# zkMIPS/zkm

Hardware: AMD Instinct MI355X
Metric: segment_proofs_per_sec (higher is better)
Workload: dtype u64 (Goldilocks p = 2^64 - 2^32 + 1, integer modular)

## Files before the change

### zkm_amd/csrc/gl_dev.h

```cpp
#pragma once
#include <stdint.h>

#if defined(__HIPCC__)
#include <hip/hip_runtime.h>
#define GL_HD __host__ __device__ __forceinline__
#else
#define GL_HD inline
#endif

typedef uint64_t gl_t;

static constexpr uint64_t GL_P = 0xFFFFFFFF00000001ULL;
static constexpr uint64_t GL_EPS = 0xFFFFFFFFULL;
static constexpr uint64_t GL_GENERATOR = 14293326489335486720ULL;
static constexpr uint64_t GL_POW2_GENERATOR = 7277203076849721926ULL;

GL_HD gl_t gl_canon(uint64_t x) { return x >= GL_P ? x - GL_P : x; }

GL_HD gl_t gl_add(gl_t a, gl_t b) {
    uint64_t s = a + b;
    return (s < a || s >= GL_P) ? s - GL_P : s;
}
GL_HD gl_t gl_sub(gl_t a, gl_t b) { return a >= b ? a - b : a - b + GL_P; }
GL_HD gl_t gl_neg(gl_t a) { return a ? GL_P - a : 0; }
// ... 71 lines not shown
    return d;
}
#endif

template <uint32_t IMM>
GL_HD uint64_t gl_mad_imm(uint32_t x, uint64_t c) {
    static_assert(IMM <= 64, "gl_mad_imm: the multiplier must be an inline constant");
#if defined(__HIP_DEVICE_COMPILE__)
    uint64_t r, carry;
    asm("v_mad_u64_u32 %0, %1, %2, %3, %4" : "=v"(r), "=s"(carry) : "v"(x), "n"(IMM), "v"(c));
    return r;
#else
    return (uint64_t)x * IMM + c;
#endif
}
template <uint32_t IMM>
GL_HD uint64_t gl_mad_imm_sc(uint32_t x, uint64_t c) {
    static_assert(IMM <= 64, "gl_mad_imm_sc: the multiplier must be an inline constant");
#if defined(__HIP_DEVICE_COMPILE__)
    uint64_t r, carry;
    asm("v_mad_u64_u32 %0, %1, %2, %3, %4" : "=v"(r), "=s"(carry) : "v"(x), "n"(IMM), "s"(c));
    return r;
#else
    return (uint64_t)x * IMM + c;
#endif
}
GL_HD uint64_t gl_mad_s(uint32_t x, uint32_t m, uint64_t c) {
#if defined(__HIP_DEVICE_COMPILE__)
    uint64_t r, carry;
    asm("v_mad_u64_u32 %0, %1, %2, %3, %4" : "=v"(r), "=s"(carry) : "v"(x), "s"(m), "v"(c));
    return r;
#else
    return (uint64_t)x * m + c;
#endif
}

GL_HD uint64_t gl_reduce128(uint64_t lo, uint64_t hi) {
    uint32_t h1 = (uint32_t)(hi >> 32), h0 = (uint32_t)hi;
#if defined(__HIP_DEVICE_COMPILE__) && !defined(GL_REDUCE_BRANCHFREE)
    uint32_t tl, th;
    uint64_t bm;
    asm("v_sub_co_u32 %0, vcc, %3, %5\n\tv_subbrev_co_u32 %1, vcc, 0, %4, vcc\n\ts_mov_b64 %2, vcc"
        : "=&v"(tl), "=&v"(th), "=s"(bm)
        : "v"((uint32_t)lo), "v"((uint32_t)(lo >> 32)), "v"(h1)
        : "vcc");
    uint64_t t0 = ((uint64_t)th << 32) | tl;
    if (__builtin_expect(bm != 0, 0)) {
        asm volatile("; ZKM_COLD");
        if ((bm >> (__lane_id() & 63)) & 1) t0 -= GL_EPS;
    }
#else
    uint64_t t0 = lo - h1;
    uint32_t m = (uint32_t)((int32_t)((uint32_t)(t0 >> 32) & ~(uint32_t)(lo >> 32)) >> 31);
    t0 -= m;
#endif
#if defined(__HIP_DEVICE_COMPILE__)
    uint64_t r, carry;
    uint32_t wrap;
    asm("v_mad_u64_u32 %0, %1, %3, -1, %4\n\ts_nop 1\n\tv_cndmask_b32 %2, 0, -1, %1" : "=&v"(r), "=&s"(carry), "=v"(wrap) : "v"(h0), "v"(t0));
    return r + wrap;
#else
    uint64_t r = (uint64_t)h0 * 0xFFFFFFFFu + t0;
    r += (r < t0) ? GL_EPS : 0;
    return r;
#endif
}
// ... 176 lines not shown
```

### zkm_amd/csrc/hash.hip

```cpp
#include <atomic>
#include "poseidon_dev.h"
#include "poseidon_lat_dev.h"
#include "poseidon_mfma_dev.h"
#include "hash_constants_dev.h"
#include "zkm_internal.h"

#ifndef ZKM_LEAF_MFMA_WAVES
#define ZKM_LEAF_MFMA_WAVES (ZKM_MFMA_PARK ? 5 : 4)
#endif

#ifndef ZKM_LATENCY_PRIO
#define ZKM_LATENCY_PRIO 3
#endif
#define ZKM_RAISE_PRIO()                                              \
    do {                                                              \
        if (ZKM_LATENCY_PRIO) __builtin_amdgcn_s_setprio(ZKM_LATENCY_PRIO); \
    } while (0)

__global__ __launch_bounds__(256) void k_poseidon_permute(gl_t* states, size_t k) {
    size_t i = (size_t)blockIdx.x * blockDim.x + threadIdx.x;
    if (i >= k) return;
    uint64_t s[12];
#pragma unroll
    for (int j = 0; j < 12; j++) s[j] = states[i * 12 + j];
    poseidon_permute(s);
#pragma unroll
    for (int j = 0; j < 12; j++) states[i * 12 + j] = s[j];
}

void zkm_launch_poseidon_permute(zkm_ctx* c, gl_t* states, size_t k) {
    if (!k) return;
    zkm_prof_scope ps(c, "poseidon_permute");
    hipLaunchKernelGGL(k_poseidon_permute, dim3((k + 255) / 256), dim3(256), 0, c->stream, states, k);
    ZKM_HIP_CHECK(hipGetLastError());
}

struct leaf_cols {
    static constexpr bool WHOLE = false;
    const gl_t* lde;
    size_t ncols, col_stride, seg;
    __device__ __forceinline__ void seek(size_t k) { lde += (size_t)blockIdx.z * seg; lde += k; }
    __device__ __forceinline__ size_t words() const { return ncols; }
    __device__ __forceinline__ uint64_t word(size_t m) const { return lde[m * col_stride]; }
};
struct leaf_f2 {
    static constexpr bool WHOLE = true;
    const gl_t* c0;
    const gl_t* c1;
    unsigned arity;
    size_t seg;
    __device__ __forceinline__ void seek(size_t k) {
        c0 += (size_t)blockIdx.z * seg; c1 += (size_t)blockIdx.z * seg;
        c0 += k * arity; c1 += k * arity;
    }
    __device__ __forceinline__ unsigned words() const { return 2 * arity; }
    __device__ __forceinline__ uint64_t word(unsigned m) const {
        const gl_t *a = c0, *b = c1;
        return ((m & 1) ? b : a)[m >> 1];
    }
};


template <class MDS>
struct sponge_lane {
    static constexpr unsigned LANES = 1;
    static constexpr bool MFMA = std::is_same<MDS, poseidon_mds_mfma>::value;
    typedef uint64_t state_t[12];
    MDS mds;
    size_t item;
    bool live;
    __device__ __forceinline__ sponge_lane() {
        if constexpr (MFMA) {
            mds.A = poseidon_mfma_operand();
#if ZKM_MFMA_PARK
            __shared__ uint32_t park[24 * ZKM_MFMA_PARK_STRIDE];
            mds.park = park + threadIdx.x;
#endif
        }
    }
    __device__ __forceinline__ bool take(size_t n) {
        item = (size_t)blockIdx.x * blockDim.x + threadIdx.x;
        live = item < n;
        if (!MFMA && !live) return false;
        if (!live) item = n - 1;
        return true;
    }
    __device__ __forceinline__ void clear(state_t& s) const {
#pragma unroll
        for (int i = 0; i < 12; i++) s[i] = 0;
    }
    template <bool RAGGED, class Src, class I>
    __device__ __forceinline__ void load(state_t& s, const Src& src, I c, I n) const {
        if (!RAGGED) {
            uint64_t v[8];
#pragma unroll
            for (int i = 0; i < 8; i++) v[i] = src.word(c + i);
#pragma unroll
            for (int i = 0; i < 8; i++) s[i] = v[i];
        } else {
#pragma unroll
            for (int i = 0; i < 8; i++)
                if ((I)i < n - c) s[i] = src.word(c + i);
        }
    }
    __device__ __forceinline__ void permute(state_t& s, int out) const { poseidon_permute_out_t(s, out, mds); }
    template <class Src>
    __device__ __forceinline__ void copy(state_t& s, const Src& src) const {
        for (size_t c = 0; c < src.words(); c++) s[c] = src.word(c);
    }
    template <class K>
    __device__ __forceinline__ void store_digest(const state_t& s, uint64_t* digests, K k, bool on) const {
        if (!on) return;
        uint64_t* d = digests + 4 * k;
        *reinterpret_cast<ulonglong2*>(d) = make_ulonglong2(s[0], s[1]);
        *reinterpret_cast<ulonglong2*>(d + 2) = make_ulonglong2(s[2], s[3]);
    }
    __device__ __forceinline__ void load_state(state_t& s, const gl_t* __restrict__ state, size_t n) const {
#pragma unroll
        for (int i = 0; i < 12; i++) s[i] = state[(size_t)i * n + item];
    }
    __device__ __forceinline__ void store_state(const state_t& s, gl_t* __restrict__ state, size_t n) const {
        if (!live) return;
#pragma unroll
        for (int i = 0; i < 12; i++) state[(size_t)i * n + item] = s[i];
    }
};

using sponge_lane_valu = sponge_lane<poseidon_mds_valu>;
using sponge_lane_mfma = sponge_lane<poseidon_mds_mfma>;

struct sponge_quad {
    static constexpr unsigned LANES = 4;
    typedef uint64_t state_t[3];
    const poseidon_quad Q;
    const unsigned q;
    size_t item;
    bool live;
    __device__ __forceinline__ sponge_quad() : Q(threadIdx.x, table()), q(threadIdx.x & 3) {}
// ... 26 lines not shown
        if (on) digests[4 * k + q] = s[0];
    }
};

struct sponge_wide {
    static constexpr unsigned LANES = 16;
    typedef uint64_t state_t[1];
    const unsigned lane, idx;
    size_t item;
    bool live;
    __device__ __forceinline__ sponge_wide() : lane(threadIdx.x & 63), idx(lane & 15) {}
    __device__ __forceinline__ bool take(size_t n) {
        item = ((size_t)blockIdx.x * blockDim.x + threadIdx.x) >> 4;
        live = item < n;
        return true;
    }
    __device__ __forceinline__ void clear(state_t& s) const { s[0] = 0; }
    template <bool RAGGED, class Src, class I>
    __device__ __forceinline__ void load(state_t& s, const Src& src, I c, I n) const {
        if (live && idx < 8 && (!RAGGED || c + idx < n)) s[0] = src.word(c + idx);
    }
    __device__ __forceinline__ void permute(state_t& s, int) const { s[0] = poseidon_permute_wide(s[0], lane); }
    template <class K>
    __device__ __forceinline__ void compress(state_t& s, const uint64_t* nodes, K k, bool on) const {
        s[0] = (on && idx < 8) ? nodes[8 * k + idx] : 0;
        permute(s, POSEIDON_OUT_DIGEST);
    }
    template <class K>
    __device__ __forceinline__ void store_digest(const state_t& s, uint64_t* digests, K k, bool on) const {
        if (on && idx < 4) digests[4 * k + idx] = s[0];
    }
};

template <class Form, class Src, bool CHUNK = false>
__device__ __forceinline__ void merkle_leaves_body(Src src, size_t n, gl_t* __restrict__ digests, size_t dig_seg, gl_t* __restrict__ state = nullptr,
                                                   int first = 1, int last = 1) {
    Form f;
    if (!f.take(n)) return;
    src.seek(f.item);
    digests += (size_t)blockIdx.z * dig_seg;
    typename Form::state_t s;
    if constexpr (CHUNK) {
        if (first) f.clear(s);
        else f.load_state(s, state, n);
    } else {
        f.clear(s);
    }
    const auto nw = src.words();
    constexpr bool NOOP = Form::LANES == 1 && !CHUNK && !Src::WHOLE;
    if (NOOP && nw <= 4) {
        if constexpr (NOOP) f.copy(s, src);
    } else {
        decltype(src.words()) c = 0;
        for (; CHUNK ? c + 8 <= nw : c < nw; c += 8) {
            if (Src::WHOLE || CHUNK || (Form::LANES == 1 && nw - c >= 8)) f.template load<false>(s, src, c, nw);
            else f.template load<true>(s, src, c, nw);
            f.permute(s, c + 16 <= nw ? POSEIDON_OUT_CAPACITY : ((Src::WHOLE || c + 8 >= nw) && !CHUNK ? POSEIDON_OUT_DIGEST : POSEIDON_OUT_ALL));
        }
        if constexpr (CHUNK) {
            if (c < nw) {
                f.template load<true>(s, src, c, nw);
                sponge_lane_valu().permute(s, POSEIDON_OUT_ALL);
            }
        }
    }
    if constexpr (CHUNK) {
        if (!last) {
            f.store_state(s, state, n);
            return;
        }
    }
    f.store_digest(s, digests, f.item, f.live);
}

#define ZKM_LEAF_MFMA_ATTR __attribute__((amdgpu_waves_per_eu(ZKM_LEAF_MFMA_WAVES, ZKM_LEAF_MFMA_WAVES)))
#define ZKM_LANE_WAVES_ATTR(n) __attribute__((amdgpu_waves_per_eu(n, n)))

__global__ __launch_bounds__(256) ZKM_LANE_WAVES_ATTR(5) void k_merkle_leaves(const gl_t* __restrict__ lde, size_t nrows, size_t ncols, size_t col_stride,
                                                       gl_t* __restrict__ digests, size_t lde_seg, size_t dig_seg) {
    merkle_leaves_body<sponge_lane_valu>(leaf_cols{lde, ncols, col_stride, lde_seg}, nrows, digests, dig_seg);
}
__global__ __launch_bounds__(256) ZKM_LEAF_MFMA_ATTR void k_merkle_leaves_mfma(const gl_t* __restrict__ lde, size_t nrows, size_t ncols, size_t col_stride,
                                                                              gl_t* __restrict__ digests, size_t lde_seg, size_t dig_seg) {
    merkle_leaves_body<sponge_lane_mfma>(leaf_cols{lde, ncols, col_stride, lde_seg}, nrows, digests, dig_seg);
}
__global__ __launch_bounds__(256) void k_merkle_leaves_quad(const gl_t* __restrict__ lde, size_t nrows, size_t ncols, size_t col_stride,
                                                            gl_t* __restrict__ digests, size_t lde_seg, size_t dig_seg) {
    ZKM_RAISE_PRIO();
    merkle_leaves_body<sponge_quad>(leaf_cols{lde, ncols, col_stride, lde_seg}, nrows, digests, dig_seg);
}
__global__ __launch_bounds__(256) void k_merkle_leaves_wide(const gl_t* __restrict__ lde, size_t nrows, size_t ncols, size_t col_stride,
                                                            gl_t* __restrict__ digests, size_t lde_seg, size_t dig_seg) {
    ZKM_RAISE_PRIO();
    merkle_leaves_body<sponge_wide>(leaf_cols{lde, ncols, col_stride, lde_seg}, nrows, digests, dig_seg);
}

__global__ __launch_bounds__(256) void k_merkle_leaves_chunk(const gl_t* __restrict__ lde, size_t nrows, size_t nc, size_t col_stride,
                                                             gl_t* __restrict__ state, int first, int last, gl_t* __restrict__ digests) {
    merkle_leaves_body<sponge_lane_valu, leaf_cols, true>(leaf_cols{lde, nc, col_stride, 0}, nrows, digests, 0, state, first, last);
}
__global__ __launch_bounds__(256) ZKM_LEAF_MFMA_ATTR void k_merkle_leaves_chunk_mfma(const gl_t* __restrict__ lde, size_t nrows, size_t nc, size_t col_stride,
                                                                                    gl_t* __restrict__ state, int first, int last, gl_t* __restrict__ digests) {
    merkle_leaves_body<sponge_lane_mfma, leaf_cols, true>(leaf_cols{lde, nc, col_stride, 0}, nrows, digests, 0, state, first, last);
}

__global__ __launch_bounds__(256) ZKM_LANE_WAVES_ATTR(5) void k_merkle_leaves_ext(const gl_t* __restrict__ c0, const gl_t* __restrict__ c1,
                                                           size_t nleaves, unsigned arity, gl_t* __restrict__ digests, size_t val_seg, size_t dig_seg) {
    merkle_leaves_body<sponge_lane_valu>(leaf_f2{c0, c1, arity, val_seg}, nleaves, digests, dig_seg);
}
__global__ __launch_bounds__(256) ZKM_LEAF_MFMA_ATTR void k_merkle_leaves_ext_mfma(const gl_t* __restrict__ c0, const gl_t* __restrict__ c1, size_t nleaves,
                                                                                  unsigned arity, gl_t* __restrict__ digests, size_t val_seg, size_t dig_seg) {
    merkle_leaves_body<sponge_lane_mfma>(leaf_f2{c0, c1, arity, val_seg}, nleaves, digests, dig_seg);
}
__global__ __launch_bounds__(256) void k_merkle_leaves_ext_quad(const gl_t* __restrict__ c0, const gl_t* __restrict__ c1, size_t nleaves,
                                                                unsigned arity, gl_t* __restrict__ digests, size_t val_seg, size_t dig_seg) {
    ZKM_RAISE_PRIO();
    merkle_leaves_body<sponge_quad>(leaf_f2{c0, c1, arity, val_seg}, nleaves, digests, dig_seg);
}
__global__ __launch_bounds__(256) void k_merkle_leaves_ext_wide(const gl_t* __restrict__ c0, const gl_t* __restrict__ c1, size_t nleaves,
                                                                unsigned arity, gl_t* __restrict__ digests, size_t val_seg, size_t dig_seg) {
    ZKM_RAISE_PRIO();
    merkle_leaves_body<sponge_wide>(leaf_f2{c0, c1, arity, val_seg}, nleaves, digests, dig_seg);
}

enum merkle_form { MERKLE_LANE, MERKLE_LANE_MFMA, MERKLE_QUAD, MERKLE_WIDE };
static merkle_form merkle_pick_form(const zkm_ctx* c, size_t hashes, bool mfma_ok) {
    if (hashes <= c->wide_max_hashes) return MERKLE_WIDE;
    if (hashes <= c->quad_max_hashes) return MERKLE_QUAD;
    return mfma_ok && c->leaf_mfma ? MERKLE_LANE_MFMA : MERKLE_LANE;
}
static dim3 leaf_grid(merkle_form f, size_t n, size_t nseg = 1) {
    static const unsigned lanes[] = {1, 1, 4, 16};
    return dim3((unsigned)((n * lanes[f] + 255) / 256), 1, (unsigned)nseg);
}

void zkm_launch_merkle_leaves(zkm_ctx* c, const gl_t* lde, size_t nrows, size_t ncols, size_t col_stride, gl_t* digests, size_t nseg,
                              size_t lde_seg, size_t dig_seg) {
    zkm_prof_scope ps(c, ncols <= 4 ? "merkle_leaves_copy" : "merkle_leaves");
    if (nseg == 0 || nseg > 65535) throw std::runtime_error("merkle_leaves: bad segment count");
    static constexpr decltype(&k_merkle_leaves) kernel[] = {k_merkle_leaves, k_merkle_leaves_mfma, k_merkle_leaves_quad, k_merkle_leaves_wide};
    const merkle_form f = ncols > 4 ? merkle_pick_form(c, nrows * nseg, true) : MERKLE_LANE;
    hipLaunchKernelGGL(kernel[f], leaf_grid(f, nrows, nseg), dim3(256), 0, c->stream, lde, nrows, ncols, col_stride, digests, lde_seg, dig_seg);
    ZKM_HIP_CHECK(hipGetLastError());
}

void zkm_launch_merkle_leaves_chunk(zkm_ctx* c, const gl_t* lde, size_t nrows, size_t nc, size_t col_stride, gl_t* state, bool first,
                                    bool last, gl_t* digests) {
    if (!last && nc % 8) throw std::runtime_error("merkle_leaves_chunk: only the last chunk may hold a ragged group of columns");
    zkm_prof_scope ps(c, "merkle_leaves");
    hipLaunchKernelGGL(c->leaf_mfma ? k_merkle_leaves_chunk_mfma : k_merkle_leaves_chunk, leaf_grid(MERKLE_LANE, nrows), dim3(256), 0, c->stream, lde, nrows,
                       nc, col_stride, state, first ? 1 : 0, last ? 1 : 0, digests);
    ZKM_HIP_CHECK(hipGetLastError());
}

void zkm_launch_merkle_leaves_ext(zkm_ctx* c, const gl_t* c0, const gl_t* c1, size_t nleaves, unsigned arity, gl_t* digests, size_t nseg,
                                  size_t val_seg, size_t dig_seg) {
    if (arity % 4 || 2 * arity <= 4) throw std::runtime_error("merkle_leaves_ext: unsupported arity");
    if (nseg == 0 || nseg > 65535) throw std::runtime_error("merkle_leaves_ext: bad segment count");
    zkm_prof_scope ps(c, "merkle_leaves_ext");
    static constexpr decltype(&k_merkle_leaves_ext) kernel[] = {k_merkle_leaves_ext, k_merkle_leaves_ext_mfma, k_merkle_leaves_ext_quad, k_merkle_leaves_ext_wide};
    const merkle_form f = merkle_pick_form(c, nleaves * nseg, true);
    hipLaunchKernelGGL(kernel[f], leaf_grid(f, nleaves, nseg), dim3(256), 0, c->stream, c0, c1, nleaves, arity, digests, val_seg, dig_seg);
    ZKM_HIP_CHECK(hipGetLastError());
}

struct merkle_fused_args {
    const gl_t* children;
    gl_t* parents[3];
    uint32_t levels;
    size_t dig_seg;
};

__global__ __launch_bounds__(256) ZKM_LANE_WAVES_ATTR(6) void k_merkle_fused(merkle_fused_args p) {
    __shared__ uint64_t sh[2][4][256];
    const unsigned tid = threadIdx.x;
    uint64_t s[12];
    {
        const ulonglong2* ch = reinterpret_cast<const ulonglong2*>(p.children + (size_t)blockIdx.z * p.dig_seg + 8 * ((size_t)blockIdx.x * 256 + tid));
        ulonglong2 a = ch[0], b = ch[1], cc = ch[2], d = ch[3];
        s[0] = a.x; s[1] = a.y; s[2] = b.x; s[3] = b.y; s[4] = cc.x; s[5] = cc.y; s[6] = d.x; s[7] = d.y;
    }
#pragma unroll 1
    for (unsigned lvl = 0; lvl < p.levels; lvl++) {
        const unsigned width = 256u >> lvl;
        if (lvl) {
#pragma unroll
            for (int w = 0; w < 4; w++) {
                s[w] = sh[(lvl - 1) & 1][w][2 * tid];
                s[4 + w] = sh[(lvl - 1) & 1][w][2 * tid + 1];
            }
        }
#pragma unroll
        for (int w = 8; w < 12; w++) s[w] = 0;
        poseidon_permute_out(s, POSEIDON_OUT_DIGEST);
        uint64_t* o = p.parents[lvl] + (size_t)blockIdx.z * p.dig_seg + 4 * ((size_t)blockIdx.x * width + tid);
// ... 417 lines not shown
```

### zkm_amd/csrc/poseidon_dev.h

```cpp
#pragma once
#include "gl_dev.h"

#undef ZKM_CONSTEXPR
#define ZKM_CONSTEXPR static constexpr
namespace pc_host {
#undef ZKM_CONST
#define ZKM_CONST static const
#include "poseidon_constants.inc"
#include "poseidon_group4.inc"
ZKM_CONST uint64_t ZKM_POSEIDON_ZERO12[12] = {0, 0, 0, 0, 0, 0, 0, 0, 0, 0, 0, 0};
}
#if defined(__HIPCC__)
namespace pc_dev {
#undef ZKM_CONST
#define ZKM_CONST static __device__ __constant__ const
#include "poseidon_constants.inc"
#include "poseidon_group4.inc"
ZKM_CONST uint64_t ZKM_POSEIDON_ZERO12[12] = {0, 0, 0, 0, 0, 0, 0, 0, 0, 0, 0, 0};
}
#endif
#undef ZKM_CONST
#undef ZKM_CONSTEXPR

#if defined(__HIP_DEVICE_COMPILE__)
#define PC pc_dev
#define POSEIDON_SCHED_FENCE() __builtin_amdgcn_sched_barrier(0)
#define POSEIDON_REGION(name) asm volatile("; ZKM_REGION " name)
#else
#define PC pc_host
#define POSEIDON_SCHED_FENCE() ((void)0)
#define POSEIDON_REGION(name) ((void)0)
#endif

#if defined(__HIP_DEVICE_COMPILE__)
#define POSEIDON_OPAQUE(c) asm("" : "+s"(c))
#define POSEIDON_OPAQUE_PTR(p) asm volatile("" : "+s"(p))
#else
#define POSEIDON_OPAQUE(c) ((void)0)
#define POSEIDON_OPAQUE_PTR(p) ((void)0)
#endif

GL_HD uint64_t poseidon_sbox7(uint64_t x) {
    uint64_t x2 = gl_mul_loose(x, x);
    uint64_t x4 = gl_mul_loose(x2, x2);
    uint64_t x3 = gl_mul_loose(x, x2);
    return gl_mul_loose(x3, x4);
}

GL_HD uint64_t poseidon_fold(uint64_t al, uint64_t ah) {
#if defined(__HIP_DEVICE_COMPILE__)
    const uint64_t t = (uint64_t)(uint32_t)(ah >> 32) * 0xFFFFFFFFu + al;
    uint32_t rhi, wrap;
    uint64_t carry;
    asm("v_add_co_u32_e64 %0, %1, %3, %4\n\ts_nop 1\n\tv_cndmask_b32 %2, 0, -1, %1"
        : "=&v"(rhi), "=&s"(carry), "=v"(wrap)
        : "v"((uint32_t)(t >> 32)), "v"((uint32_t)ah));
    return (((uint64_t)rhi << 32) | (uint32_t)t) + wrap;
#endif
    uint64_t s1 = (uint64_t)(uint32_t)(ah >> 32) * 0xFFFFFFFFu + al;
    uint64_t hs = (uint64_t)(uint32_t)ah + (s1 >> 32);
    uint64_t base = (hs << 32) | (uint32_t)s1;
    return (uint64_t)(uint32_t)(hs >> 32) * 0xFFFFFFFFu + base;
}

GL_HD uint64_t gl_mad_s_co(uint32_t x, uint32_t m, uint64_t c, uint64_t& carry) {
#if defined(__HIP_DEVICE_COMPILE__)
    uint64_t r;
    asm("v_mad_u64_u32 %0, %1, %2, %3, %4" : "=v"(r), "=s"(carry) : "v"(x), "s"(m), "v"(c));
    return r;
#else
    const uint64_t r = (uint64_t)x * m + c;
    carry = r < c;
// ... 50 lines not shown
    POSEIDON_OPAQUE(diag);
#pragma unroll
    for (int r = ROW0; r < ROW1; r++) {
        uint64_t al = ADD ? gl_mad_imm_sc<17>(lo[r], (uint64_t)(uint32_t)add[r]) : 0, ah = ADD ? gl_mad_imm_sc<17>(hi[r], add[r] >> 32) : 0;
#pragma unroll
        for (int i = ADD ? 1 : 0; i < 12; i++) {
            al += (uint64_t)lo[(i + r) % 12] * C[i];
            ah += (uint64_t)hi[(i + r) % 12] * C[i];
        }
        if (r == 0) {
            al += (uint64_t)lo[0] * diag;
            ah += (uint64_t)hi[0] * diag;
        }
        s[r] = poseidon_fold(al, ah);
        if ((r & 3) == 3) POSEIDON_SCHED_FENCE();
    }
}
GL_HD void poseidon_mds(uint64_t s[12]) { poseidon_mds_add<false>(s, nullptr); }

GL_HD uint64_t poseidon_sbox_delta(uint64_t a) { return gl_sub_rr(poseidon_sbox7(a), a); }
GL_HD constexpr uint32_t poseidon_m1(int i, int j) {
    constexpr uint32_t C[12] = {17, 15, 41, 16, 2, 28, 13, 13, 39, 18, 34, 20};
    return C[(j - i + 12) % 12] + ((i == 0 && j == 0) ? 8u : 0u);
}

template <int J>
GL_HD void poseidon_m_row0(const uint32_t lo[12], const uint32_t hi[12], uint64_t& al, uint64_t& ah) {
    if constexpr (J < 12) {
        al = gl_mad_imm<poseidon_m1(0, J)>(lo[J], al);
        ah = gl_mad_imm<poseidon_m1(0, J)>(hi[J], ah);
        poseidon_m_row0<J + 1>(lo, hi, al, ah);
    }
}
template <int T, int I>
GL_HD void poseidon_group_rows(uint64_t s[12], const uint32_t lo[12], const uint32_t hi[12], uint32_t d1l, uint32_t d1h, uint32_t d2l, uint32_t d2h,
                               const uint64_t* c3) {
    if constexpr (I < 12) {
        uint64_t al, ah;
        if (T == 3) {
            al = gl_mad_s(d1l, PC::ZKM_POSEIDON_M2[I][0], gl_mad_imm_sc<poseidon_m1(I, 0)>(d2l, (uint64_t)(uint32_t)c3[I]));
            ah = gl_mad_s(d1h, PC::ZKM_POSEIDON_M2[I][0], gl_mad_imm_sc<poseidon_m1(I, 0)>(d2h, c3[I] >> 32));
#pragma unroll
            for (int j = 0; j < 12; j++) {
                al = gl_mad_s(lo[j], PC::ZKM_POSEIDON_M3[I][j], al);
                ah = gl_mad_s(hi[j], PC::ZKM_POSEIDON_M3[I][j], ah);
            }
        } else {
            al = gl_mad_imm_sc<poseidon_m1(I, 0)>(d1l, (uint64_t)(uint32_t)c3[I]);
            ah = gl_mad_imm_sc<poseidon_m1(I, 0)>(d1h, c3[I] >> 32);
#pragma unroll
            for (int j = 0; j < 12; j++) {
                al = gl_mad_s(lo[j], PC::ZKM_POSEIDON_M2[I][j], al);
                ah = gl_mad_s(hi[j], PC::ZKM_POSEIDON_M2[I][j], ah);
            }
        }
        s[I] = poseidon_fold(al, ah);
        if ((I & 1) == 1) POSEIDON_SCHED_FENCE();
        poseidon_group_rows<T, I + 1>(s, lo, hi, d1l, d1h, d2l, d2h, c3);
    }
}

template <int I>
GL_HD void poseidon_group4_rows(uint64_t s[12], const uint32_t lo[12], const uint32_t hi[12], uint32_t d1l, uint32_t d1h, uint32_t d2l, uint32_t d2h,
                                uint32_t d3l, uint32_t d3h, const uint64_t* c4) {
    if constexpr (I < 12) {
        static_assert(PC::ZKM_POSEIDON_G4_DCOL[0][I] == poseidon_m1(I, 0) && PC::ZKM_POSEIDON_G4_DCOL[1][I] == PC::ZKM_POSEIDON_M2[I][0] &&
                      PC::ZKM_POSEIDON_G4_DCOL[2][I] == PC::ZKM_POSEIDON_M3[I][0], "first columns of M, M^2, M^3");
        uint64_t al = gl_mad_imm_sc<poseidon_m1(I, 0)>(d3l, (uint64_t)(uint32_t)c4[I]), ah = gl_mad_imm_sc<poseidon_m1(I, 0)>(d3h, c4[I] >> 32);
        al = gl_mad_s(d2l, PC::ZKM_POSEIDON_G4_DCOL[1][I], al);
        ah = gl_mad_s(d2h, PC::ZKM_POSEIDON_G4_DCOL[1][I], ah);
        al = gl_mad_s(d1l, PC::ZKM_POSEIDON_G4_DCOL[2][I], al);
        ah = gl_mad_s(d1h, PC::ZKM_POSEIDON_G4_DCOL[2][I], ah);
#pragma unroll
        for (int j = 0; j < 11; j++) {
            al = gl_mad_s(lo[j], PC::ZKM_POSEIDON_M4[I][j], al);
            ah = gl_mad_s(hi[j], PC::ZKM_POSEIDON_M4[I][j], ah);
        }
        uint64_t cl, ch;
        al = gl_mad_s_co(lo[11], PC::ZKM_POSEIDON_M4[I][11], al, cl);
        ah = gl_mad_s_co(hi[11], PC::ZKM_POSEIDON_M4[I][11], ah, ch);
        s[I] = poseidon_fold_wide(al, ah, cl, ch);
        if ((I & 1) == 1) POSEIDON_SCHED_FENCE();
        poseidon_group4_rows<I + 1>(s, lo, hi, d1l, d1h, d2l, d2h, d3l, d3h, c4);
    }
}

template <int T, bool ROW0_ASM = true, class DELTA>
GL_HD void poseidon_partial_group_t(uint64_t s[12], uint64_t c1, uint64_t c2, const uint64_t* c3, DELTA&& delta, const uint64_t* c4 = nullptr) {
    static_assert(T == 2 || T == 3 || T == 4, "groups of two, three or four layers");
    uint32_t lo[12], hi[12];
#pragma unroll
    for (int i = 0; i < 12; i++) {
        lo[i] = (uint32_t)s[i];
        hi[i] = (uint32_t)(s[i] >> 32);
    }
    uint64_t al = gl_mad_imm_sc<poseidon_m1(0, 0)>(lo[0], (uint64_t)(uint32_t)c1), ah = gl_mad_imm_sc<poseidon_m1(0, 0)>(hi[0], c1 >> 32);
    if constexpr (ROW0_ASM) {
        poseidon_m_row0<1>(lo, hi, al, ah);
    } else {
#pragma unroll
        for (int j = 1; j < 12; j++) {
            al += (uint64_t)lo[j] * poseidon_m1(0, j);
            ah += (uint64_t)hi[j] * poseidon_m1(0, j);
        }
    }
    const uint64_t d1 = delta(0, poseidon_fold(al, ah));
    const uint32_t d1l = (uint32_t)d1, d1h = (uint32_t)(d1 >> 32);
    uint32_t d2l = 0, d2h = 0;
    POSEIDON_SCHED_FENCE();
    if (T >= 3) {
        al = gl_mad_imm_sc<poseidon_m1(0, 0)>(d1l, (uint64_t)(uint32_t)c2);
        ah = gl_mad_imm_sc<poseidon_m1(0, 0)>(d1h, c2 >> 32);
#pragma unroll
        for (int j = 0; j < 12; j++) {
            al = gl_mad_s(lo[j], PC::ZKM_POSEIDON_M2[0][j], al);
            ah = gl_mad_s(hi[j], PC::ZKM_POSEIDON_M2[0][j], ah);
        }
        const uint64_t d2 = delta(1, poseidon_fold(al, ah));
        d2l = (uint32_t)d2;
        d2h = (uint32_t)(d2 >> 32);
        POSEIDON_SCHED_FENCE();
    }
    if constexpr (T == 4) {
        al = gl_mad_s(d1l, PC::ZKM_POSEIDON_M2[0][0], gl_mad_imm_sc<poseidon_m1(0, 0)>(d2l, (uint64_t)(uint32_t)c3[0]));
        ah = gl_mad_s(d1h, PC::ZKM_POSEIDON_M2[0][0], gl_mad_imm_sc<poseidon_m1(0, 0)>(d2h, c3[0] >> 32));
#pragma unroll
        for (int j = 0; j < 12; j++) {
            al = gl_mad_s(lo[j], PC::ZKM_POSEIDON_M3[0][j], al);
            ah = gl_mad_s(hi[j], PC::ZKM_POSEIDON_M3[0][j], ah);
        }
        const uint64_t d3 = delta(2, poseidon_fold(al, ah));
        POSEIDON_SCHED_FENCE();
        poseidon_group4_rows<0>(s, lo, hi, d1l, d1h, d2l, d2h, (uint32_t)d3, (uint32_t)(d3 >> 32), c4);
    } else {
        poseidon_group_rows<T, 0>(s, lo, hi, d1l, d1h, d2l, d2h, c3);
    }
}
GL_HD void poseidon_partial_group4(uint64_t s[12], uint64_t c1, uint64_t c2, const uint64_t* c3, const uint64_t* c4) {
    poseidon_partial_group_t<4>(s, c1, c2, c3, [](int, uint64_t a) { return poseidon_sbox_delta(a); }, c4);
}
template <int T>
GL_HD void poseidon_partial_group(uint64_t s[12], uint64_t c1, uint64_t c2, const uint64_t* c3) {
    poseidon_partial_group_t<T>(s, c1, c2, c3, [](int, uint64_t a) { return poseidon_sbox_delta(a); });
}

enum { POSEIDON_OUT_ALL = 0, POSEIDON_OUT_CAPACITY = 1, POSEIDON_OUT_DIGEST = 2 };

struct poseidon_mds_valu {
    GL_HD void layer(uint64_t s[12], int next) const {
        poseidon_mds_add<true>(s, next < 30 ? &PC::ZKM_POSEIDON_RC[next * 12] : PC::ZKM_POSEIDON_ZERO12);
    }
};

template <class MDS>
GL_HD void poseidon_permute_out_t(uint64_t s[12], int out, const MDS& mds) {
    POSEIDON_REGION("entry");
    const uint64_t* rc0 = PC::ZKM_POSEIDON_RC;
    POSEIDON_OPAQUE_PTR(rc0);
#pragma unroll
    for (int i = 0; i < 12; i++) s[i] = gl_add_lc(s[i], rc0[i]);
#pragma unroll 1
    for (int r = 0; r < 8; r++) {
        POSEIDON_REGION("full_sbox");
#pragma unroll
        for (int i = 0; i < 12; i++) {
            s[i] = poseidon_sbox7(s[i]);
            if ((i & 1) == 1) POSEIDON_SCHED_FENCE();
        }
        if (r == 3) {
            POSEIDON_REGION("partial_head");
#pragma unroll 1
            for (int g = 0; g < 5; g++) {
                POSEIDON_REGION("partial_group4");
                poseidon_partial_group4(s, PC::ZKM_POSEIDON_G4_C1[g], PC::ZKM_POSEIDON_G4_C2[g], &PC::ZKM_POSEIDON_G4_C3[g], PC::ZKM_POSEIDON_G4_C4[g]);
                s[0] = poseidon_sbox7(s[0]);
            }
            POSEIDON_REGION("partial_tail");
            const uint64_t* tc12 = PC::ZKM_POSEIDON_G4_TAIL_C12;
            const uint64_t* tc3 = PC::ZKM_POSEIDON_G4_TAIL_C3;
            POSEIDON_OPAQUE_PTR(tc12);
            POSEIDON_OPAQUE_PTR(tc3);
            poseidon_partial_group<3>(s, tc12[0], tc12[1], tc3);
        } else if (r == 7 && out != POSEIDON_OUT_ALL) {
            POSEIDON_REGION("last_mds_rows");
            if (out == POSEIDON_OUT_CAPACITY) poseidon_mds_add<false, 8, 12>(s, nullptr);
            else poseidon_mds_add<false, 0, 4>(s, nullptr);
        } else {
            POSEIDON_REGION("full_mds");
            const int next = (r < 3 ? r : 22 + r) + 1;
            mds.layer(s, next);
        }
    }
    POSEIDON_REGION("exit");
    if (out == POSEIDON_OUT_ALL) {
#pragma unroll
        for (int i = 0; i < 12; i++) s[i] = gl_canon(s[i]);
    } else if (out == POSEIDON_OUT_DIGEST) {
#pragma unroll
        for (int i = 0; i < 4; i++) s[i] = gl_canon(s[i]);
    }
}

GL_HD void poseidon_permute_out(uint64_t s[12], int out) { poseidon_permute_out_t(s, out, poseidon_mds_valu{}); }

GL_HD void poseidon_permute(uint64_t s[12]) { poseidon_permute_out(s, POSEIDON_OUT_ALL); }
```

Before: 17.90.

## Reread kernel args from kernarg segment and use literal MDS multipliers in Poseidon

Kernel parameters are packed into structs and, for per-lane sponges, re-read through the kernarg segment pointer instead of being held in registers across the permutation. The per-lane item index is recomputed after hashing. Partial-round MDS row products now use inline-asm v_mad_u64_u32 with the constant loaded by s_mov, replacing per-coefficient scalar operands. Digest-only outputs can skip the last truncated MDS rows. The aim is to cut SGPR/VGPR pressure in the leaf hashing kernels, at the cost of more fragile asm and scheduling.

Measured after the change: 17.92, median of 4. Within noise of the previous version (+0.1%).

```diff
diff --git a/zkm_amd/csrc/gl_dev.h b/zkm_amd/csrc/gl_dev.h
--- a/zkm_amd/csrc/gl_dev.h
+++ b/zkm_amd/csrc/gl_dev.h
@@ -127,6 +127,34 @@
     return r;
 #else
     return (uint64_t)x * m + c;
+#endif
+}
+template <uint32_t M>
+GL_HD void gl_mad2_lit(uint32_t xl, uint32_t xh, uint64_t& al, uint64_t& ah) {
+#if defined(__HIP_DEVICE_COMPILE__)
+    uint32_t m;
+    uint64_t carry;
+    asm("s_mov_b32 %2, %6\n\tv_mad_u64_u32 %0, %3, %4, %2, %0\n\tv_mad_u64_u32 %1, %3, %5, %2, %1"
+        : "+v"(al), "+v"(ah), "=&s"(m), "=&s"(carry)
+        : "v"(xl), "v"(xh), "n"(M));
+#else
+    al += (uint64_t)xl * M;
+    ah += (uint64_t)xh * M;
+#endif
+}
+template <uint32_t M>
+GL_HD void gl_mad2_lit_co(uint32_t xl, uint32_t xh, uint64_t& al, uint64_t& ah, uint64_t& cl, uint64_t& ch) {
+#if defined(__HIP_DEVICE_COMPILE__)
+    uint32_t m;
+    asm("s_mov_b32 %2, %7\n\tv_mad_u64_u32 %0, %3, %5, %2, %0\n\tv_mad_u64_u32 %1, %4, %6, %2, %1"
+        : "+v"(al), "+v"(ah), "=&s"(m), "=&s"(cl), "=&s"(ch)
+        : "v"(xl), "v"(xh), "n"(M));
+#else
+    const uint64_t l = al + (uint64_t)xl * M, h = ah + (uint64_t)xh * M;
+    cl = l < al;
+    ch = h < ah;
+    al = l;
+    ah = h;
 #endif
 }
 
diff --git a/zkm_amd/csrc/hash.hip b/zkm_amd/csrc/hash.hip
--- a/zkm_amd/csrc/hash.hip
+++ b/zkm_amd/csrc/hash.hip
@@ -35,29 +35,84 @@
     ZKM_HIP_CHECK(hipGetLastError());
 }
 
+#define ZKM_CONST_AS __attribute__((address_space(4)))
+template <class A, bool REREAD>
+struct kernel_args {
+    const A& held;
+    __device__ __forceinline__ explicit kernel_args(const A& a) : held(a) {}
+#if defined(__HIP_DEVICE_COMPILE__)
+    __device__ __forceinline__ auto operator->() const {
+        if constexpr (REREAD) {
+            const ZKM_CONST_AS A* p = (const ZKM_CONST_AS A*)__builtin_amdgcn_kernarg_segment_ptr();
+            asm volatile("" : "+s"(p));
+            return p;
+        } else {
+            return &held;
+        }
+    }
+#else
+    __device__ const A* operator->() const { return &held; }
+#endif
+};
+
+struct leaf_cols_args {
+    const gl_t* lde;
+    size_t n, ncols, col_stride;
+    gl_t* digests;
+    size_t lde_seg, dig_seg;
+};
+struct leaf_chunk_args {
+    const gl_t* lde;
+    size_t n, ncols, col_stride;
+    gl_t* state;
+    int first, last;
+    gl_t* digests;
+    static constexpr size_t lde_seg = 0, dig_seg = 0;
+};
+template <class KA>
 struct leaf_cols {
     static constexpr bool WHOLE = false;
-    const gl_t* lde;
-    size_t ncols, col_stride, seg;
-    __device__ __forceinline__ void seek(size_t k) { lde += (size_t)blockIdx.z * seg; lde += k; }
-    __device__ __forceinline__ size_t words() const { return ncols; }
-    __device__ __forceinline__ uint64_t word(size_t m) const { return lde[m * col_stride]; }
-};
+    const KA a;
+    const gl_t* row;
+    struct view {
+        const gl_t* row;
+        size_t col_stride;
+        __device__ __forceinline__ uint64_t word(unsigned m) const { return row[m * col_stride]; }
+    };
+    __device__ __forceinline__ explicit leaf_cols(const KA& ka) : a(ka), row(nullptr) {}
+    __device__ __forceinline__ void seek(size_t k) { row = a->lde + (size_t)blockIdx.z * a->lde_seg; row += k; }
+    __device__ __forceinline__ unsigned words() const { return (unsigned)a->ncols; }
+    __device__ __forceinline__ view open() const { return view{row, a->col_stride}; }
+    __device__ __forceinline__ uint64_t word(unsigned m) const { return row[m * a->col_stride]; }
+};
+struct leaf_f2_args {
+    const gl_t* c0;
+    const gl_t* c1;
+    size_t n;
+    unsigned arity;
+    gl_t* digests;
+    size_t val_seg, dig_seg;
+};
+template <class KA>
 struct leaf_f2 {
     static constexpr bool WHOLE = true;
+    const KA a;
     const gl_t* c0;
-    const gl_t* c1;
-    unsigned arity;
-    size_t seg;
-    __device__ __forceinline__ void seek(size_t k) {
-        c0 += (size_t)blockIdx.z * seg; c1 += (size_t)blockIdx.z * seg;
-        c0 += k * arity; c1 += k * arity;
-    }
-    __device__ __forceinline__ unsigned words() const { return 2 * arity; }
-    __device__ __forceinline__ uint64_t word(unsigned m) const {
-        const gl_t *a = c0, *b = c1;
-        return ((m & 1) ? b : a)[m >> 1];
-    }
+    struct view {
+        const gl_t* c0;
+        size_t gap;
+        __device__ __forceinline__ uint64_t word(unsigned m) const {
+            const gl_t* p = (m & 1) ? reinterpret_cast<const gl_t*>(reinterpret_cast<const char*>(c0) + gap) : c0;
+            return p[m >> 1];
+        }
+    };
+    __device__ __forceinline__ explicit leaf_f2(const KA& ka) : a(ka), c0(nullptr) {}
+    __device__ __forceinline__ void seek(size_t k) { c0 = a->c0 + (size_t)blockIdx.z * a->val_seg + k * a->arity; }
+    __device__ __forceinline__ unsigned words() const { return 2 * a->arity; }
+    __device__ __forceinline__ view open() const {
+        return view{c0, (size_t)(reinterpret_cast<uintptr_t>(a->c1) - reinterpret_cast<uintptr_t>(a->c0))};
+    }
+    __device__ __forceinline__ uint64_t word(unsigned m) const { return open().word(m); }
 };
 
 
@@ -85,6 +140,15 @@
         if (!live) item = n - 1;
         return true;
     }
+    __device__ __forceinline__ void retake(size_t n) {
+        unsigned t = threadIdx.x;
+#if defined(__HIP_DEVICE_COMPILE__)
+        asm volatile("" : "+v"(t));
+#endif
+        item = (size_t)blockIdx.x * blockDim.x + t;
+        live = item < n;
+        if (!live) item = n - 1;
+    }
     __device__ __forceinline__ void clear(state_t& s) const {
 #pragma unroll
         for (int i = 0; i < 12; i++) s[i] = 0;
@@ -92,9 +156,10 @@
     template <bool RAGGED, class Src, class I>
     __device__ __forceinline__ void load(state_t& s, const Src& src, I c, I n) const {
         if (!RAGGED) {
+            const auto w = src.open();
             uint64_t v[8];
 #pragma unroll
-            for (int i = 0; i < 8; i++) v[i] = src.word(c + i);
+            for (int i = 0; i < 8; i++) v[i] = w.word(c + i);
 #pragma unroll
             for (int i = 0; i < 8; i++) s[i] = v[i];
         } else {
@@ -103,7 +168,7 @@
                 if ((I)i < n - c) s[i] = src.word(c + i);
         }
     }
-    __device__ __forceinline__ void permute(state_t& s, int out) const { poseidon_permute_out_t(s, out, mds); }
+    __device__ __forceinline__ void permute(state_t& s, int out) const { poseidon_permute_out_t<false>(s, out, mds); }
     template <class Src>
     __device__ __forceinline__ void copy(state_t& s, const Src& src) const {
         for (size_t c = 0; c < src.words(); c++) s[c] = src.word(c);
@@ -196,30 +261,33 @@
     }
 };
 
-template <class Form, class Src, bool CHUNK = false>
-__device__ __forceinline__ void merkle_leaves_body(Src src, size_t n, gl_t* __restrict__ digests, size_t dig_seg, gl_t* __restrict__ state = nullptr,
-                                                   int first = 1, int last = 1) {
+template <class Form, template <class> class Src, bool CHUNK = false, class Args>
+__device__ __forceinline__ void merkle_leaves_body(const Args& args) {
+    typedef kernel_args<Args, Form::LANES == 1> KA;
+    const KA a(args);
     Form f;
-    if (!f.take(n)) return;
+    if (!f.take(a->n)) return;
+    Src<KA> src(a);
     src.seek(f.item);
-    digests += (size_t)blockIdx.z * dig_seg;
     typename Form::state_t s;
     if constexpr (CHUNK) {
-        if (first) f.clear(s);
-        else f.load_state(s, state, n);
+        if (a->first) f.clear(s);
+        else f.load_state(s, a->state, a->n);
     } else {
         f.clear(s);
     }
-    const auto nw = src.words();
-    constexpr bool NOOP = Form::LANES == 1 && !CHUNK && !Src::WHOLE;
+    auto nw = src.words();
+    constexpr bool WHOLE = Src<KA>::WHOLE;
+    constexpr bool NOOP = Form::LANES == 1 && !CHUNK && !WHOLE;
     if (NOOP && nw <= 4) {
         if constexpr (NOOP) f.copy(s, src);
     } else {
         decltype(src.words()) c = 0;
         for (; CHUNK ? c + 8 <= nw : c < nw; c += 8) {
-            if (Src::WHOLE || CHUNK || (Form::LANES == 1 && nw - c >= 8)) f.template load<false>(s, src, c, nw);
+            if (WHOLE || CHUNK || (Form::LANES == 1 && nw - c >= 8)) f.template load<false>(s, src, c, nw);
             else f.template load<true>(s, src, c, nw);
-            f.permute(s, c + 16 <= nw ? POSEIDON_OUT_CAPACITY : ((Src::WHOLE || c + 8 >= nw) && !CHUNK ? POSEIDON_OUT_DIGEST : POSEIDON_OUT_ALL));
+            f.permute(s, c + 16 <= nw ? POSEIDON_OUT_CAPACITY : ((WHOLE || c + 8 >= nw) && !CHUNK ? POSEIDON_OUT_DIGEST : POSEIDON_OUT_ALL));
+            nw = src.words();
         }
         if constexpr (CHUNK) {
             if (c < nw) {
@@ -228,63 +296,44 @@
             }
         }
     }
+    if constexpr (Form::LANES == 1) {
+        if constexpr (!Form::MFMA) f.retake(a->n);
+    }
     if constexpr (CHUNK) {
-        if (!last) {
-            f.store_state(s, state, n);
+        if (!a->last) {
+            f.store_state(s, a->state, a->n);
             return;
         }
     }
-    f.store_digest(s, digests, f.item, f.live);
+    f.store_digest(s, a->digests + (size_t)blockIdx.z * a->dig_seg, f.item, f.live);
 }
 
 #define ZKM_LEAF_MFMA_ATTR __attribute__((amdgpu_waves_per_eu(ZKM_LEAF_MFMA_WAVES, ZKM_LEAF_MFMA_WAVES)))
 #define ZKM_LANE_WAVES_ATTR(n) __attribute__((amdgpu_waves_per_eu(n, n)))
 
-__global__ __launch_bounds__(256) ZKM_LANE_WAVES_ATTR(5) void k_merkle_leaves(const gl_t* __restrict__ lde, size_t nrows, size_t ncols, size_t col_stride,
-                                                       gl_t* __restrict__ digests, size_t lde_seg, size_t dig_seg) {
-    merkle_leaves_body<sponge_lane_valu>(leaf_cols{lde, ncols, col_stride, lde_seg}, nrows, digests, dig_seg);
-}
-__global__ __launch_bounds__(256) ZKM_LEAF_MFMA_ATTR void k_merkle_leaves_mfma(const gl_t* __restrict__ lde, size_t nrows, size_t ncols, size_t col_stride,
-                                                                              gl_t* __restrict__ digests, size_t lde_seg, size_t dig_seg) {
-    merkle_leaves_body<sponge_lane_mfma>(leaf_cols{lde, ncols, col_stride, lde_seg}, nrows, digests, dig_seg);
-}
-__global__ __launch_bounds__(256) void k_merkle_leaves_quad(const gl_t* __restrict__ lde, size_t nrows, size_t ncols, size_t col_stride,
-                                                            gl_t* __restrict__ digests, size_t lde_seg, size_t dig_seg) {
+__global__ __launch_bounds__(256) ZKM_LANE_WAVES_ATTR(5) void k_merkle_leaves(leaf_cols_args p) { merkle_leaves_body<sponge_lane_valu, leaf_cols>(p); }
+__global__ __launch_bounds__(256) ZKM_LEAF_MFMA_ATTR void k_merkle_leaves_mfma(leaf_cols_args p) { merkle_leaves_body<sponge_lane_mfma, leaf_cols>(p); }
+__global__ __launch_bounds__(256) void k_merkle_leaves_quad(leaf_cols_args p) {
     ZKM_RAISE_PRIO();
-    merkle_leaves_body<sponge_quad>(leaf_cols{lde, ncols, col_stride, lde_seg}, nrows, digests, dig_seg);
-}
-__global__ __launch_bounds__(256) void k_merkle_leaves_wide(const gl_t* __restrict__ lde, size_t nrows, size_t ncols, size_t col_stride,
-                                                            gl_t* __restrict__ digests, size_t lde_seg, size_t dig_seg) {
+    merkle_leaves_body<sponge_quad, leaf_cols>(p);
+}
+__global__ __launch_bounds__(256) void k_merkle_leaves_wide(leaf_cols_args p) {
     ZKM_RAISE_PRIO();
-    merkle_leaves_body<sponge_wide>(leaf_cols{lde, ncols, col_stride, lde_seg}, nrows, digests, dig_seg);
-}
-
-__global__ __launch_bounds__(256) void k_merkle_leaves_chunk(const gl_t* __restrict__ lde, size_t nrows, size_t nc, size_t col_stride,
-                                                             gl_t* __restrict__ state, int first, int last, gl_t* __restrict__ digests) {
-    merkle_leaves_body<sponge_lane_valu, leaf_cols, true>(leaf_cols{lde, nc, col_stride, 0}, nrows, digests, 0, state, first, last);
-}
-__global__ __launch_bounds__(256) ZKM_LEAF_MFMA_ATTR void k_merkle_leaves_chunk_mfma(const gl_t* __restrict__ lde, size_t nrows, size_t nc, size_t col_stride,
-                                                                                    gl_t* __restrict__ state, int first, int last, gl_t* __restrict__ digests) {
-    merkle_leaves_body<sponge_lane_mfma, leaf_cols, true>(leaf_cols{lde, nc, col_stride, 0}, nrows, digests, 0, state, first, last);
-}
-
-__global__ __launch_bounds__(256) ZKM_LANE_WAVES_ATTR(5) void k_merkle_leaves_ext(const gl_t* __restrict__ c0, const gl_t* __restrict__ c1,
-                                                           size_t nleaves, unsigned arity, gl_t* __restrict__ digests, size_t val_seg, size_t dig_seg) {
-    merkle_leaves_body<sponge_lane_valu>(leaf_f2{c0, c1, arity, val_seg}, nleaves, digests, dig_seg);
-}
-__global__ __launch_bounds__(256) ZKM_LEAF_MFMA_ATTR void k_merkle_leaves_ext_mfma(const gl_t* __restrict__ c0, const gl_t* __restrict__ c1, size_t nleaves,
-                                                                                  unsigned arity, gl_t* __restrict__ digests, size_t val_seg, size_t dig_seg) {
-    merkle_leaves_body<sponge_lane_mfma>(leaf_f2{c0, c1, arity, val_seg}, nleaves, digests, dig_seg);
-}
-__global__ __launch_bounds__(256) void k_merkle_leaves_ext_quad(const gl_t* __restrict__ c0, const gl_t* __restrict__ c1, size_t nleaves,
-                                                                unsigned arity, gl_t* __restrict__ digests, size_t val_seg, size_t dig_seg) {
+    merkle_leaves_body<sponge_wide, leaf_cols>(p);
+}
+
+__global__ __launch_bounds__(256) void k_merkle_leaves_chunk(leaf_chunk_args p) { merkle_leaves_body<sponge_lane_valu, leaf_cols, true>(p); }
+__global__ __launch_bounds__(256) ZKM_LEAF_MFMA_ATTR void k_merkle_leaves_chunk_mfma(leaf_chunk_args p) { merkle_leaves_body<sponge_lane_mfma, leaf_cols, true>(p); }
+
+__global__ __launch_bounds__(256) ZKM_LANE_WAVES_ATTR(5) void k_merkle_leaves_ext(leaf_f2_args p) { merkle_leaves_body<sponge_lane_valu, leaf_f2>(p); }
+__global__ __launch_bounds__(256) ZKM_LEAF_MFMA_ATTR void k_merkle_leaves_ext_mfma(leaf_f2_args p) { merkle_leaves_body<sponge_lane_mfma, leaf_f2>(p); }
+__global__ __launch_bounds__(256) void k_merkle_leaves_ext_quad(leaf_f2_args p) {
     ZKM_RAISE_PRIO();
-    merkle_leaves_body<sponge_quad>(leaf_f2{c0, c1, arity, val_seg}, nleaves, digests, dig_seg);
-}
-__global__ __launch_bounds__(256) void k_merkle_leaves_ext_wide(const gl_t* __restrict__ c0, const gl_t* __restrict__ c1, size_t nleaves,
-                                                                unsigned arity, gl_t* __restrict__ digests, size_t val_seg, size_t dig_seg) {
+    merkle_leaves_body<sponge_quad, leaf_f2>(p);
+}
+__global__ __launch_bounds__(256) void k_merkle_leaves_ext_wide(leaf_f2_args p) {
     ZKM_RAISE_PRIO();
-    merkle_leaves_body<sponge_wide>(leaf_f2{c0, c1, arity, val_seg}, nleaves, digests, dig_seg);
+    merkle_leaves_body<sponge_wide, leaf_f2>(p);
 }
 
 enum merkle_form { MERKLE_LANE, MERKLE_LANE_MFMA, MERKLE_QUAD, MERKLE_WIDE };
@@ -302,18 +351,20 @@
                               size_t lde_seg, size_t dig_seg) {
     zkm_prof_scope ps(c, ncols <= 4 ? "merkle_leaves_copy" : "merkle_leaves");
     if (nseg == 0 || nseg > 65535) throw std::runtime_error("merkle_leaves: bad segment count");
+    if (ncols > 0xFFFFFFF0u) throw std::runtime_error("merkle_leaves: too many columns");
     static constexpr decltype(&k_merkle_leaves) kernel[] = {k_merkle_leaves, k_merkle_leaves_mfma, k_merkle_leaves_quad, k_merkle_leaves_wide};
     const merkle_form f = ncols > 4 ? merkle_pick_form(c, nrows * nseg, true) : MERKLE_LANE;
-    hipLaunchKernelGGL(kernel[f], leaf_grid(f, nrows, nseg), dim3(256), 0, c->stream, lde, nrows, ncols, col_stride, digests, lde_seg, dig_seg);
+    hipLaunchKernelGGL(kernel[f], leaf_grid(f, nrows, nseg), dim3(256), 0, c->stream, leaf_cols_args{lde, nrows, ncols, col_stride, digests, lde_seg, dig_seg});
     ZKM_HIP_CHECK(hipGetLastError());
 }
 
 void zkm_launch_merkle_leaves_chunk(zkm_ctx* c, const gl_t* lde, size_t nrows, size_t nc, size_t col_stride, gl_t* state, bool first,
                                     bool last, gl_t* digests) {
     if (!last && nc % 8) throw std::runtime_error("merkle_leaves_chunk: only the last chunk may hold a ragged group of columns");
+    if (nc > 0xFFFFFFF0u) throw std::runtime_error("merkle_leaves_chunk: too many columns");
     zkm_prof_scope ps(c, "merkle_leaves");
-    hipLaunchKernelGGL(c->leaf_mfma ? k_merkle_leaves_chunk_mfma : k_merkle_leaves_chunk, leaf_grid(MERKLE_LANE, nrows), dim3(256), 0, c->stream, lde, nrows,
-                       nc, col_stride, state, first ? 1 : 0, last ? 1 : 0, digests);
+    hipLaunchKernelGGL(c->leaf_mfma ? k_merkle_leaves_chunk_mfma : k_merkle_leaves_chunk, leaf_grid(MERKLE_LANE, nrows), dim3(256), 0, c->stream,
+                       leaf_chunk_args{lde, nrows, nc, col_stride, state, first ? 1 : 0, last ? 1 : 0, digests});
     ZKM_HIP_CHECK(hipGetLastError());
 }
 
@@ -324,7 +375,7 @@
     zkm_prof_scope ps(c, "merkle_leaves_ext");
     static constexpr decltype(&k_merkle_leaves_ext) kernel[] = {k_merkle_leaves_ext, k_merkle_leaves_ext_mfma, k_merkle_leaves_ext_quad, k_merkle_leaves_ext_wide};
     const merkle_form f = merkle_pick_form(c, nleaves * nseg, true);
-    hipLaunchKernelGGL(kernel[f], leaf_grid(f, nleaves, nseg), dim3(256), 0, c->stream, c0, c1, nleaves, arity, digests, val_seg, dig_seg);
+    hipLaunchKernelGGL(kernel[f], leaf_grid(f, nleaves, nseg), dim3(256), 0, c->stream, leaf_f2_args{c0, c1, nleaves, arity, digests, val_seg, dig_seg});
     ZKM_HIP_CHECK(hipGetLastError());
 }
 
diff --git a/zkm_amd/csrc/poseidon_dev.h b/zkm_amd/csrc/poseidon_dev.h
--- a/zkm_amd/csrc/poseidon_dev.h
+++ b/zkm_amd/csrc/poseidon_dev.h
@@ -34,10 +34,12 @@
 
 #if defined(__HIP_DEVICE_COMPILE__)
 #define POSEIDON_OPAQUE(c) asm("" : "+s"(c))
-#define POSEIDON_OPAQUE_PTR(p) asm volatile("" : "+s"(p))
+#define POSEIDON_TABLE_PTR(name, table)                                                                            \
+    const __attribute__((address_space(4))) uint64_t* name = (const __attribute__((address_space(4))) uint64_t*)(table); \
+    asm volatile("" : "+s"(name))
 #else
 #define POSEIDON_OPAQUE(c) ((void)0)
-#define POSEIDON_OPAQUE_PTR(p) ((void)0)
+#define POSEIDON_TABLE_PTR(name, table) const uint64_t* name = (table)
 #endif
 
 GL_HD uint64_t poseidon_sbox7(uint64_t x) {
@@ -154,12 +156,26 @@
         poseidon_m_row0<J + 1>(lo, hi, al, ah);
     }
 }
-template <int T, int I>
+template <int P, int I, int J, int N>
+GL_HD void poseidon_row_terms(const uint32_t lo[12], const uint32_t hi[12], uint64_t& al, uint64_t& ah) {
+    static_assert(P == 2 || P == 3 || P == 4, "powers of the MDS matrix with tables");
+    if constexpr (J < N) {
+        constexpr uint32_t m = P == 2 ? PC::ZKM_POSEIDON_M2[I][J] : P == 3 ? PC::ZKM_POSEIDON_M3[I][J] : PC::ZKM_POSEIDON_M4[I][J];
+        gl_mad2_lit<m>(lo[J], hi[J], al, ah);
+        poseidon_row_terms<P, I, J + 1, N>(lo, hi, al, ah);
+    }
+}
+template <int T, bool LIT, int I, class C3>
 GL_HD void poseidon_group_rows(uint64_t s[12], const uint32_t lo[12], const uint32_t hi[12], uint32_t d1l, uint32_t d1h, uint32_t d2l, uint32_t d2h,
-                               const uint64_t* c3) {
+                               const C3 c3) {
     if constexpr (I < 12) {
         uint64_t al, ah;
-        if (T == 3) {
+        if constexpr (LIT) {
+            al = gl_mad_imm_sc<poseidon_m1(I, 0)>(T == 3 ? d2l : d1l, (uint64_t)(uint32_t)c3[I]);
+            ah = gl_mad_imm_sc<poseidon_m1(I, 0)>(T == 3 ? d2h : d1h, c3[I] >> 32);
+            if constexpr (T == 3) gl_mad2_lit<PC::ZKM_POSEIDON_M2[I][0]>(d1l, d1h, al, ah);
+            poseidon_row_terms<T, I, 0, 12>(lo, hi, al, ah);
+        } else if (T == 3) {
             al = gl_mad_s(d1l, PC::ZKM_POSEIDON_M2[I][0], gl_mad_imm_sc<poseidon_m1(I, 0)>(d2l, (uint64_t)(uint32_t)c3[I]));
             ah = gl_mad_s(d1h, PC::ZKM_POSEIDON_M2[I][0], gl_mad_imm_sc<poseidon_m1(I, 0)>(d2h, c3[I] >> 32));
 #pragma unroll
@@ -178,37 +194,30 @@
         }
         s[I] = poseidon_fold(al, ah);
         if ((I & 1) == 1) POSEIDON_SCHED_FENCE();
-        poseidon_group_rows<T, I + 1>(s, lo, hi, d1l, d1h, d2l, d2h, c3);
-    }
-}
-
-template <int I>
+        poseidon_group_rows<T, LIT, I + 1>(s, lo, hi, d1l, d1h, d2l, d2h, c3);
+    }
+}
+
+template <int I, class C4>
 GL_HD void poseidon_group4_rows(uint64_t s[12], const uint32_t lo[12], const uint32_t hi[12], uint32_t d1l, uint32_t d1h, uint32_t d2l, uint32_t d2h,
-                                uint32_t d3l, uint32_t d3h, const uint64_t* c4) {
+                                uint32_t d3l, uint32_t d3h, const C4 c4) {
     if constexpr (I < 12) {
         static_assert(PC::ZKM_POSEIDON_G4_DCOL[0][I] == poseidon_m1(I, 0) && PC::ZKM_POSEIDON_G4_DCOL[1][I] == PC::ZKM_POSEIDON_M2[I][0] &&
                       PC::ZKM_POSEIDON_G4_DCOL[2][I] == PC::ZKM_POSEIDON_M3[I][0], "first columns of M, M^2, M^3");
         uint64_t al = gl_mad_imm_sc<poseidon_m1(I, 0)>(d3l, (uint64_t)(uint32_t)c4[I]), ah = gl_mad_imm_sc<poseidon_m1(I, 0)>(d3h, c4[I] >> 32);
-        al = gl_mad_s(d2l, PC::ZKM_POSEIDON_G4_DCOL[1][I], al);
-        ah = gl_mad_s(d2h, PC::ZKM_POSEIDON_G4_DCOL[1][I], ah);
-        al = gl_mad_s(d1l, PC::ZKM_POSEIDON_G4_DCOL[2][I], al);
-        ah = gl_mad_s(d1h, PC::ZKM_POSEIDON_G4_DCOL[2][I], ah);
-#pragma unroll
-        for (int j = 0; j < 11; j++) {
-            al = gl_mad_s(lo[j], PC::ZKM_POSEIDON_M4[I][j], al);
-            ah = gl_mad_s(hi[j], PC::ZKM_POSEIDON_M4[I][j], ah);
-        }
+        gl_mad2_lit<PC::ZKM_POSEIDON_G4_DCOL[1][I]>(d2l, d2h, al, ah);
+        gl_mad2_lit<PC::ZKM_POSEIDON_G4_DCOL[2][I]>(d1l, d1h, al, ah);
+        poseidon_row_terms<4, I, 0, 11>(lo, hi, al, ah);
         uint64_t cl, ch;
-        al = gl_mad_s_co(lo[11], PC::ZKM_POSEIDON_M4[I][11], al, cl);
-        ah = gl_mad_s_co(hi[11], PC::ZKM_POSEIDON_M4[I][11], ah, ch);
+        gl_mad2_lit_co<PC::ZKM_POSEIDON_M4[I][11]>(lo[11], hi[11], al, ah, cl, ch);
         s[I] = poseidon_fold_wide(al, ah, cl, ch);
         if ((I & 1) == 1) POSEIDON_SCHED_FENCE();
         poseidon_group4_rows<I + 1>(s, lo, hi, d1l, d1h, d2l, d2h, d3l, d3h, c4);
     }
 }
 
-template <int T, bool ROW0_ASM = true, class DELTA>
-GL_HD void poseidon_partial_group_t(uint64_t s[12], uint64_t c1, uint64_t c2, const uint64_t* c3, DELTA&& delta, const uint64_t* c4 = nullptr) {
+template <int T, bool ROW0_ASM = true, class DELTA, class C3, class C4 = const uint64_t*>
+GL_HD void poseidon_partial_group_t(uint64_t s[12], uint64_t c1, uint64_t c2, const C3 c3, DELTA&& delta, const C4 c4 = nullptr) {
     static_assert(T == 2 || T == 3 || T == 4, "groups of two, three or four layers");
     uint32_t lo[12], hi[12];
 #pragma unroll
@@ -233,10 +242,14 @@
     if (T >= 3) {
         al = gl_mad_imm_sc<poseidon_m1(0, 0)>(d1l, (uint64_t)(uint32_t)c2);
         ah = gl_mad_imm_sc<poseidon_m1(0, 0)>(d1h, c2 >> 32);
-#pragma unroll
-        for (int j = 0; j < 12; j++) {
-            al = gl_mad_s(lo[j], PC::ZKM_POSEIDON_M2[0][j], al);
-            ah = gl_mad_s(hi[j], PC::ZKM_POSEIDON_M2[0][j], ah);
+        if constexpr (ROW0_ASM) {
+            poseidon_row_terms<2, 0, 0, 12>(lo, hi, al, ah);
+        } else {
+#pragma unroll
+            for (int j = 0; j < 12; j++) {
+                al = gl_mad_s(lo[j], PC::ZKM_POSEIDON_M2[0][j], al);
+                ah = gl_mad_s(hi[j], PC::ZKM_POSEIDON_M2[0][j], ah);
+            }
         }
         const uint64_t d2 = delta(1, poseidon_fold(al, ah));
         d2l = (uint32_t)d2;
@@ -244,25 +257,22 @@
         POSEIDON_SCHED_FENCE();
     }
     if constexpr (T == 4) {
-        al = gl_mad_s(d1l, PC::ZKM_POSEIDON_M2[0][0], gl_mad_imm_sc<poseidon_m1(0, 0)>(d2l, (uint64_t)(uint32_t)c3[0]));
-        ah = gl_mad_s(d1h, PC::ZKM_POSEIDON_M2[0][0], gl_mad_imm_sc<poseidon_m1(0, 0)>(d2h, c3[0] >> 32));
-#pragma unroll
-        for (int j = 0; j < 12; j++) {
-            al = gl_mad_s(lo[j], PC::ZKM_POSEIDON_M3[0][j], al);
-            ah = gl_mad_s(hi[j], PC::ZKM_POSEIDON_M3[0][j], ah);
-        }
+        al = gl_mad_imm_sc<poseidon_m1(0, 0)>(d2l, (uint64_t)(uint32_t)c3[0]);
+        ah = gl_mad_imm_sc<poseidon_m1(0, 0)>(d2h, c3[0] >> 32);
+        gl_mad2_lit<PC::ZKM_POSEIDON_M2[0][0]>(d1l, d1h, al, ah);
+        poseidon_row_terms<3, 0, 0, 12>(lo, hi, al, ah);
         const uint64_t d3 = delta(2, poseidon_fold(al, ah));
         POSEIDON_SCHED_FENCE();
         poseidon_group4_rows<0>(s, lo, hi, d1l, d1h, d2l, d2h, (uint32_t)d3, (uint32_t)(d3 >> 32), c4);
     } else {
-        poseidon_group_rows<T, 0>(s, lo, hi, d1l, d1h, d2l, d2h, c3);
+        poseidon_group_rows<T, ROW0_ASM, 0>(s, lo, hi, d1l, d1h, d2l, d2h, c3);
     }
 }
 GL_HD void poseidon_partial_group4(uint64_t s[12], uint64_t c1, uint64_t c2, const uint64_t* c3, const uint64_t* c4) {
     poseidon_partial_group_t<4>(s, c1, c2, c3, [](int, uint64_t a) { return poseidon_sbox_delta(a); }, c4);
 }
-template <int T>
-GL_HD void poseidon_partial_group(uint64_t s[12], uint64_t c1, uint64_t c2, const uint64_t* c3) {
+template <int T, class C3>
+GL_HD void poseidon_partial_group(uint64_t s[12], uint64_t c1, uint64_t c2, const C3 c3) {
     poseidon_partial_group_t<T>(s, c1, c2, c3, [](int, uint64_t a) { return poseidon_sbox_delta(a); });
 }
 
@@ -274,11 +284,10 @@
     }
 };
 
-template <class MDS>
+template <bool DIGEST_ROWS = true, class MDS>
 GL_HD void poseidon_permute_out_t(uint64_t s[12], int out, const MDS& mds) {
     POSEIDON_REGION("entry");
-    const uint64_t* rc0 = PC::ZKM_POSEIDON_RC;
-    POSEIDON_OPAQUE_PTR(rc0);
+    POSEIDON_TABLE_PTR(rc0, PC::ZKM_POSEIDON_RC);
 #pragma unroll
     for (int i = 0; i < 12; i++) s[i] = gl_add_lc(s[i], rc0[i]);
 #pragma unroll 1
@@ -298,13 +307,12 @@
                 s[0] = poseidon_sbox7(s[0]);
             }
             POSEIDON_REGION("partial_tail");
-            const uint64_t* tc12 = PC::ZKM_POSEIDON_G4_TAIL_C12;
-            const uint64_t* tc3 = PC::ZKM_POSEIDON_G4_TAIL_C3;
-            POSEIDON_OPAQUE_PTR(tc12);
-            POSEIDON_OPAQUE_PTR(tc3);
+            POSEIDON_TABLE_PTR(tc12, PC::ZKM_POSEIDON_G4_TAIL_C12);
+            POSEIDON_TABLE_PTR(tc3, PC::ZKM_POSEIDON_G4_TAIL_C3);
             poseidon_partial_group<3>(s, tc12[0], tc12[1], tc3);
-        } else if (r == 7 && out != POSEIDON_OUT_ALL) {
+        } else if (r == 7 && (out == POSEIDON_OUT_CAPACITY || (DIGEST_ROWS && out == POSEIDON_OUT_DIGEST))) {
             POSEIDON_REGION("last_mds_rows");
+            POSEIDON_SCHED_FENCE();
             if (out == POSEIDON_OUT_CAPACITY) poseidon_mds_add<false, 8, 12>(s, nullptr);
             else poseidon_mds_add<false, 0, 4>(s, nullptr);
         } else {
```
